# christoskokas/gtsam-vSLAM

Hardware: AMD Instinct MI355X
Metric: frames/sec (extract+match+localBA), 1500 feat stereo 752x480 (higher is better)
Workload: dtype u8/i32 (extract, match) + f64 (pose LM, local BA)

## Files before the change

### gtsam-vslam_amd/csrc/extract_kernels.hpp

```cpp
#pragma once
#include "common.hpp"

namespace vslam {

struct PyrDesc {
    int nLevels;
    int w[MAX_LEVELS], h[MAX_LEVELS], pitch[MAX_LEVELS];
    uint32_t off[MAX_LEVELS];
    uint32_t imgStride;
};

struct FastDesc {
    int minXY;
    int edge3;
    int nCols[MAX_LEVELS], nRows[MAX_LEVELS], gridW[MAX_LEVELS], gridH[MAX_LEVELS];
    int cellBase[MAX_LEVELS + 1];
    int cellCap;
    int tileRows, tilePitch;
};

struct BlurDesc {
    int tilesX[MAX_LEVELS];
    int tileBase[MAX_LEVELS + 1];
    int taps[7];
// ... 15 lines not shown
constexpr int FAST_TILE_MAX = 76;
constexpr int BLUR_RPT = 16;
constexpr int BLUR_TW = 256, BLUR_TH = 4 * BLUR_RPT;

void launch_load_images(hipStream_t s, const uint8_t* const* dSrc, int stride, uint8_t* pyr, const PyrDesc& P, int nimg);
void launch_load_images_color(hipStream_t s, const uint8_t* const* dSrc, int stride, int channels, uint8_t* pyr, const PyrDesc& P,
                              int nimg);
struct RectSrc {
    const uint8_t* src; const float* mapX; const float* mapY;
    int sw, sh, stride, pad;
};
void launch_load_images_rect(hipStream_t s, const RectSrc* dTab, int channels, uint8_t* pyr, const PyrDesc& P, int nimg);
void launch_resize(hipStream_t s, uint8_t* pyr, const PyrDesc& P, int level, const int2* xtab,
                   const int2* ytab, int nimg);
void launch_fast(hipStream_t s, const uint8_t* pyr, const PyrDesc& P, const FastDesc& F,
                 uint32_t* cellSlots, int* cellCount, int maxThr, int minThr, int nimg);
#ifdef VSLAM_FAST_CHECK
int fast_check_failures(hipStream_t s);
#endif
void launch_gather(hipStream_t s, const uint32_t* cellSlots, const int* cellCount, const FastDesc& F,
                   int nLevels, int* cellOff, uint32_t* cand, int candCap, int* levelCount, int nimg);
void launch_blur(hipStream_t s, const uint8_t* pyr, uint8_t* blur, const PyrDesc& P,
                 const BlurDesc& B, int nimg);
struct DiscRows { int umax[16]; };
void launch_orient_desc(hipStream_t s, const uint8_t* pyr, const uint8_t* blur, const PyrDesc& P,
                        const LevelTables& T, const uint32_t* kept, const int* keptOff, int keptCap,
                        const DiscRows& disc, vslam_keypoint* kps, uint8_t* desc, int outCap,
                        int maxKept, int nimg);
void upload_pattern();

constexpr int SSC_NMAX_LDS = 16384;
constexpr int SSC_NMAX = 65535;
constexpr int SSC_PICKW_G = 2048;
struct SscArgs {
    const uint32_t* cand; int candCap; const int* levelCount;
    int nLevels, nimg;
    int numRet[MAX_LEVELS], cols[MAX_LEVELS], rows[MAX_LEVELS], high[MAX_LEVELS], kmin[MAX_LEVELS], kmax[MAX_LEVELS];
    uint32_t* tmp;
    uint32_t* gridG;
    const size_t* gridOff;
    uint32_t* aG; uint32_t* sortedG; uint32_t* picksG;
    int forceGlobal;
    int* taskCount;
    int* flags;
};

void launch_ssc(hipStream_t s, const SscArgs& A, uint32_t* kept, int keptCap, int* keptOff, int* hostCounts);

}
```

### gtsam-vslam_amd/csrc/extractor.hip

```cpp
#include "extractor.hpp"
#include <atomic>
#include <algorithm>
#include <cmath>
#include <mutex>

namespace vslam {

static thread_local char g_err[512] = "";
void set_error(const char* fmt, ...) {
    va_list ap;
    va_start(ap, fmt);
    vsnprintf(g_err, sizeof(g_err), fmt, ap);
    va_end(ap);
}

}

using namespace vslam;

static void build_fe_tables(vslam_extractor& e) {
    const int nL = e.nLevels;
    const vslam_fe_params& p = e.prm;
    e.scalePyramid.assign(nL, 1.f);
    e.scaleInvPyramid.assign(nL, 1.f);
// ... 183 lines not shown
    VS_HIP(hipMalloc(&d_kept, (size_t)nimg * keptCap * sizeof(uint32_t)));
    VS_HIP(hipMalloc(&d_keptOff, (size_t)nimg * (MAX_LEVELS + 1) * sizeof(int)));
    VS_HIP(hipMalloc(&d_kps, (size_t)nimg * keptCap * sizeof(vslam_keypoint)));
    VS_HIP(hipMalloc(&d_desc, (size_t)nimg * keptCap * 32));

    for (int v = 0; v < 16; v++) discRows.umax[v] = umax[v];
    nKept.assign(nimg, 0);
    for (int l = 0; l < nLevels; l++) {
        const int numRet = featurePerLevel[l], cols = P.w[l], rows = P.h[l];
        const int e1 = rows + cols + 2 * numRet;
        const long long e2 = 4LL * cols + 4LL * numRet + 4LL * rows * numRet + (long long)rows * rows +
                             (long long)cols * cols - 2LL * rows * cols + 4LL * rows * cols * numRet;
        const double e3 = std::sqrt((double)e2), e4 = numRet - 1;
        const double s1 = -std::round((e1 + e3) / e4), s2 = -std::round((e1 - e3) / e4);
        sscHigh[l] = (int)(s1 > s2 ? s1 : s2);
        const unsigned K = (unsigned)numRet;
        sscKmin[l] = (int)(unsigned)std::round((float)K - ((float)K * 0.1f));
        sscKmax[l] = (int)(unsigned)std::round((float)K + ((float)K * 0.1f));
    }
    VS_HIP(hipMalloc(&d_sscTmp, (size_t)3 * nimg * candCap * sizeof(uint32_t)));
    VS_HIP(hipMalloc(&d_sscPicks, (size_t)nimg * nLevels * 8 * SSC_PICKW_G * sizeof(uint32_t)));
    {
        size_t words = 0;
        std::vector<size_t> off((size_t)nimg * nLevels, 0);
        for (int i = 0; i < nimg; i++)
            for (int l = 0; l < nLevels; l++) {
                off[(size_t)i * nLevels + l] = words;
                words += (size_t)(2 * P.h[l] + 2) * (size_t)((2 * P.w[l] + 2 + 31) / 32);
            }
        VS_HIP(hipMalloc(&d_sscGrid, words * sizeof(uint32_t)));
        VS_HIP(hipMalloc(&d_sscGridOff, off.size() * sizeof(size_t)));
        VS_HIP(hipMemcpy(d_sscGridOff, off.data(), off.size() * sizeof(size_t), hipMemcpyHostToDevice));
    }
    VS_HIP(hipMalloc(&d_taskCount, (size_t)nimg * MAX_LEVELS * sizeof(int) + (size_t)nimg * MAX_LEVELS * 8 * sizeof(long long)));
    VS_HIP(hipMalloc(&d_sscFlags, (size_t)nimg * 2 * sizeof(int)));
    VS_HIP(vslam::memset_sync(d_sscFlags, 0, (size_t)nimg * 2 * sizeof(int)));
    VS_HIP(hipHostMalloc(&h_counts, (size_t)nimg * 3 * sizeof(int), hipHostMallocMapped));
    VS_HIP(hipHostGetDevicePointer((void**)&d_counts, h_counts, 0));
    memset(h_counts, 0, (size_t)nimg * 3 * sizeof(int));
    if (const char* e = getenv("VSLAM_SSC_FORCE_GLOBAL")) sscForceGlobal = atoi(e) != 0;
    return VSLAM_OK;
}

void vslam_extractor::release() {
    if (stream) hipStreamSynchronize(stream);
    timer.destroy();
    hipFree(d_pyr); hipFree(d_blur); hipFree(d_xtab); hipFree(d_ytab);
    hipFree(d_cellSlots); hipFree(d_cellCount); hipFree(d_cellOff);
    hipFree(d_cand); hipFree(d_levelCount);
    if (doubleOut) { hipFree(d_kpsBuf[0]); hipFree(d_kpsBuf[1]); hipFree(d_descBuf[0]); hipFree(d_descBuf[1]); }
    else { hipFree(d_kps); hipFree(d_desc); }
    hipFree(d_kept); hipFree(d_keptOff);
    hipFree(d_sscTmp); hipFree(d_sscPicks); hipFree(d_taskCount); hipFree(d_sscFlags); hipFree(d_sscGrid); hipFree(d_sscGridOff);
    d_sscGrid = nullptr; d_sscGridOff = nullptr; d_sscPicks = nullptr;
    if (h_counts) hipHostFree(h_counts);
    if (h_imgPtrs) hipHostFree(h_imgPtrs);
    hipFree(d_imgPtrs); h_imgPtrs = nullptr; d_imgPtrs = nullptr;
    if (h_colPtrs) hipHostFree(h_colPtrs);
    hipFree(d_colPtrs); hipFree(d_colStage); h_colPtrs = nullptr; d_colPtrs = nullptr; d_colStage = nullptr; colStageBytes = 0;
    if (evColPtrs) hipEventDestroy(evColPtrs);
    evColPtrs = nullptr;
    if (h_rectTab) hipHostFree(h_rectTab);
    hipFree(d_rectTab); h_rectTab = nullptr; d_rectTab = nullptr;
    if (evRectTab) hipEventDestroy(evRectTab);
    evRectTab = nullptr;
    d_sscTmp = nullptr; d_taskCount = nullptr; d_sscFlags = nullptr; h_counts = nullptr;
    if (evGather) hipEventDestroy(evGather);
// ... 138 lines not shown
        hipFree(d_colStage); d_colStage = nullptr; colStageBytes = 0;
        VS_HIP(hipMalloc((void**)&d_colStage, need));
        colStageBytes = need;
    }
    size_t at = 0;
    for (int i = 0; i < nimg; i++) {
        RectSrc& t = h_rectTab[i];
        t = RectSrc{};
        if (!ptrs[i]) continue;
        const vslam_rectifier* r = rects[i];
        t.mapX = r->d_mapX; t.mapY = r->d_mapY; t.sw = r->sw; t.sh = r->sh;
        if (srcOnDevice) { t.src = ptrs[i]; t.stride = stride; continue; }
        const int pitch = align_up(r->sw * channels, 16);
        uint8_t* dst = d_colStage + at;
        at += (size_t)r->sh * pitch;
        VS_HIP(hipMemcpy2DAsync(dst, pitch, ptrs[i], stride, (size_t)r->sw * channels, r->sh, hipMemcpyHostToDevice, stream));
        t.src = dst; t.stride = pitch;
    }
    VS_HIP(hipMemcpyAsync(d_rectTab, h_rectTab, (size_t)nimg * sizeof(RectSrc), hipMemcpyHostToDevice, stream));
    VS_HIP(hipEventRecord(evRectTab, stream));
    launch_load_images_rect(stream, d_rectTab, channels, d_pyr, P, nimg);
    VS_HIP(hipGetLastError());
    if (sync && !srcOnDevice) VS_HIP(hipStreamSynchronize(stream));
    return VSLAM_OK;
}

vslam_status vslam_extractor::wait_counts() {
    if (!countsPending) return VSLAM_OK;
    VS_HIP(hipSetDevice(device));
    VS_HIP(hipEventSynchronize(evDone));
    countsPending = false;
#ifdef VSLAM_SSC_STAMPS
    {
        std::vector<long long> st((size_t)nimg * nLevels * 8);
        hipMemcpy(st.data(), d_taskCount + nimg * MAX_LEVELS, st.size() * sizeof(long long), hipMemcpyDeviceToHost);
        for (int i = 0; i < nimg; i++) for (int l = 0; l < nLevels; l++) { const long long* q = &st[(size_t)(i * nLevels + l) * 8]; fprintf(stderr, "ssc img %d lvl %d: n %lld partitions %lld countsort %lld search %lld (probes %lld final w %lld) emit %lld\n", i, l, q[4], q[0], q[1], q[2], q[5], q[6], q[3]); }
    }
#endif
    for (int i = 0; i < nimg; i++) {
        if (h_counts[nimg + 2 * i + 1]) { set_error("FAST candidate / kept-keypoint overflow"); return VSLAM_ERR_CAPACITY; }
        if (h_counts[nimg + 2 * i]) {
            set_error("SSC: image %d exceeds a kernel limit (mask %d: 1 = more than %d candidates in one level, 4 = segment list, "
                      "8 / 32 = width search, 16 = probe grid)", i, h_counts[nimg + 2 * i], SSC_NMAX);
            return VSLAM_ERR_CAPACITY;
        }
        nKept[i] = h_counts[i];
    }
    return VSLAM_OK;
}

vslam_status vslam_extractor::enqueue_ssc() {
    SscArgs S{};
    S.cand = d_cand; S.candCap = candCap; S.levelCount = d_levelCount; S.nLevels = nLevels; S.nimg = nimg;
    for (int l = 0; l < nLevels; l++) {
        S.numRet[l] = featurePerLevel[l]; S.cols[l] = P.w[l]; S.rows[l] = P.h[l];
        S.high[l] = sscHigh[l]; S.kmin[l] = sscKmin[l]; S.kmax[l] = sscKmax[l];
    }
    S.gridG = d_sscGrid; S.gridOff = d_sscGridOff;
    S.tmp = d_sscTmp; S.aG = d_sscTmp + (size_t)nimg * candCap; S.sortedG = d_sscTmp + (size_t)2 * nimg * candCap;
    S.picksG = d_sscPicks; S.forceGlobal = sscForceGlobal ? 1 : 0;
    S.taskCount = d_taskCount; S.flags = d_sscFlags;
    launch_ssc(stream, S, d_kept, keptCap, d_keptOff, d_counts);
    return VSLAM_OK;
}

#ifdef VSLAM_HOST_STAMPS
#include <chrono>
static double hs_now() { return std::chrono::duration<double, std::micro>(std::chrono::steady_clock::now().time_since_epoch()).count(); }
#define HS(k) hs[k] = hs_now()
// ... 296 lines not shown
```

### gtsam-vslam_amd/csrc/ssc.hip

```cpp
#include "extract_kernels.hpp"
#include <mutex>

namespace vslam {

constexpr int SSC_NT = 512, SSC_NW = SSC_NT / 64;
constexpr int SSC_NPROBE = 8;
constexpr int SSC_COOP_MIN = 2048;
constexpr int SSC_ARENA_WORDS = 20 * 1024;
constexpr int SSC_NMAX_SMALL = 6144;

template <int M> struct SscCfg;
template <> struct SscCfg<0> { static constexpr int NMAX = SSC_NMAX_LDS, SEGMAX = 1088, PICKW = SSC_NMAX_LDS / 32, ARENA = SSC_ARENA_WORDS; };
template <> struct SscCfg<1> { static constexpr int NMAX = SSC_NMAX, SEGMAX = 4096, PICKW = SSC_PICKW_G, ARENA = SSC_ARENA_WORDS; };
template <> struct SscCfg<2> { static constexpr int NMAX = SSC_NMAX_SMALL, SEGMAX = 1088, PICKW = SSC_NMAX_SMALL / 32, ARENA = 10 * 1024; };

template <bool G> __device__ __forceinline__ void ssc_fence() {
    if (G) asm volatile("s_waitcnt vmcnt(0) lgkmcnt(0)" ::: "memory");
    else asm volatile("s_waitcnt lgkmcnt(0)" ::: "memory");
}
__device__ __forceinline__ void ssc_lds_fence() { asm volatile("s_waitcnt lgkmcnt(0)" ::: "memory"); }

__device__ __forceinline__ int ssc_cell(int v, int width, float rcpw) {
    const int t = 2 * v;
    int q = (int)((float)t * rcpw);
    q -= (q * width > t);
    q += ((q + 1) * width <= t);
    return q;
}

template <bool G>
__device__ __forceinline__ int ssc_eval(const uint32_t* sc, int n, int width, int cols, int rows, uint32_t* grid, int gridWords,
                                        uint32_t* picks, bool& fits, int abortAbove) {
    const int lane = threadIdx.x & 63;
    const float rcpw = 1.0f / (float)width;
    const int gc = ssc_cell(cols, width, rcpw), gr = ssc_cell(rows, width, rcpw);
    const int span = 2;
    const int rowWords = (gc + 1 + 31) >> 5;
    const int words = (gr + 1) * rowWords;
    fits = words <= gridWords;
    if (!fits) return -1;
    for (int i = lane; i < words; i += 64) grid[i] = 0;
    ssc_lds_fence();
    asm volatile("s_waitcnt vmcnt(0)" ::: "memory");
    int count = 0;
    uint32_t pkNext = lane < n ? sc[lane] : 0u;
    for (int base = 0; base < n; base += 64) {
        const int i = base + lane;
        const bool valid = i < n;
        const uint32_t pk = pkNext;
        if (G) pkNext = (i + 64 < n) ? sc[i + 64] : 0u;
        const int row = ssc_cell(cand_y(pk), width, rcpw);
        const int col = ssc_cell(cand_x(pk), width, rcpw);
        bool covered = true;
        if (valid) covered = (grid[row * rowWords + (col >> 5)] >> (col & 31)) & 1u;
        unsigned long long pend = __ballot(!covered), picked = 0ull;
        while (pend) {
            const int l = __ffsll((long long)pend) - 1;
            picked |= 1ull << l;
            const int rl = __builtin_amdgcn_readlane(row, l), cl = __builtin_amdgcn_readlane(col, l);
            const bool conflict = abs(row - rl) <= span && abs(col - cl) <= span;
            pend &= ~__ballot(conflict);
        }
        if ((picked >> lane) & 1ull) {
            const int r0 = max(row - span, 0), r1 = min(row + span, gr);
            const int c0 = max(col - span, 0), c1 = min(col + span, gc);
            const int w0 = c0 >> 5, w1 = c1 >> 5;
            for (int rr = r0; rr <= r1; rr++) {
                if (w0 == w1) {
                    const uint32_t m = ((1u << (c1 - c0 + 1)) - 1u) << (c0 & 31);
                    atomicOr(&grid[rr * rowWords + w0], m);
                } else {
                    atomicOr(&grid[rr * rowWords + w0], 0xffffffffu << (c0 & 31));
                    atomicOr(&grid[rr * rowWords + w1], 0xffffffffu >> (31 - (c1 & 31)));
                }
            }
        }
        if (picks && lane < 2) picks[(base >> 5) + lane] = (uint32_t)(picked >> (32 * lane));
        count += __popcll(picked);
        if (!G) pkNext = (i + 64 < n) ? sc[i + 64] : 0u;
        ssc_lds_fence();
        asm volatile("s_waitcnt vmcnt(0)" ::: "memory");
        if (abortAbove >= 0 && count > abortAbove) break;
    }
    return count;
}

constexpr int SSC_LONGMAX = 64;
__device__ int g_sscCoopMin = SSC_COOP_MIN;
__device__ __forceinline__ void ssc_push(uint32_t* segN, int* cntN, int segMax, int f, int e, int depth, int* sFail) {
    if (e - f > g_sscCoopMin) {
        const int q = atomicAdd(cntN + 2, 1);
        if (q < SSC_LONGMAX) { segN[2 * q] = (uint32_t)f | ((uint32_t)e << 16); segN[2 * q + 1] = (uint32_t)depth; }
        else *sFail = 4;
        return;
    }
    const int q = atomicAdd(cntN, 1) + SSC_LONGMAX;
    if (q < segMax) { segN[2 * q] = (uint32_t)f | ((uint32_t)e << 16); segN[2 * q + 1] = (uint32_t)depth; }
    else *sFail = 4;
}

template <bool G>
__device__ void ssc_adjust_heap(uint32_t* first, int holeIndex, int len, uint32_t value) {
    const int topIndex = holeIndex;
    int secondChild = holeIndex;
    while (secondChild < (len - 1) / 2) {
        secondChild = 2 * (secondChild + 1);
        if ((first[secondChild] >> 16) < (first[secondChild - 1] >> 16)) secondChild--;
        first[holeIndex] = first[secondChild];
        ssc_fence<G>();
        holeIndex = secondChild;
    }
    if ((len & 1) == 0 && secondChild == (len - 2) / 2) {
        secondChild = 2 * (secondChild + 1);
        first[holeIndex] = first[secondChild - 1];
// ... 11 lines not shown
    ssc_fence<G>();
}
template <bool G>
__device__ void ssc_heapsort(uint32_t* first, int len) {
    if (len < 2) return;
    for (int parent = (len - 2) / 2;; parent--) {
        const uint32_t value = first[parent];
        ssc_adjust_heap<G>(first, parent, len, value);
        if (parent == 0) break;
    }
    for (int last = len; last > 1;) {
        --last;
        const uint32_t value = first[last];
        first[last] = first[0];
        ssc_fence<G>();
        ssc_adjust_heap<G>(first, 0, last, value);
    }
}

__device__ __forceinline__ int ssc_sel_lo(unsigned long long m, int k) {
    unsigned w = (unsigned)m;
    int pos = 0;
    const int cl = __popc(w);
    if (k >= cl) { k -= cl; w = (unsigned)(m >> 32); pos = 32; }
#pragma unroll
    for (int s = 16; s >= 1; s >>= 1) {
        const unsigned lowmask = (1u << s) - 1u;
        const int c = __popc(w & lowmask);
        if (k >= c) { k -= c; w >>= s; pos += s; } else w &= lowmask;
    }
    return pos;
}

template <bool G>
__device__ __forceinline__ void ssc_small_segment(uint32_t* a, int f, int e, int depth, uint16_t* Lp, uint16_t* Rp,
                                                  uint32_t* segN, int* cntN, int segMax, int* sFail) {
    const int lane = threadIdx.x & 63, m = e - f;
    uint32_t v = lane < m ? a[f + lane] : 0u;
    int lo = lane < m ? 0 : 64, hi = lane < m ? m : 64, d = depth;
    for (;;) {
        const bool act = (hi - lo) > 16;
        if (__ballot(act) == 0ull) break;
        if (__ballot(act && d == 0) != 0ull) {
            if (lane < m) a[f + lane] = v;
            if (act && lane == lo) ssc_push(segN, cntN, segMax, f + lo, f + hi, d, sFail);
            ssc_fence<G>();
            return;
        }
        const int ia = act ? lo + 1 : lane, ib = act ? lo + (hi - lo) / 2 : lane, ic = act ? hi - 1 : lane;
        const uint32_t va = __shfl(v, ia), vb = __shfl(v, ib), vc = __shfl(v, ic), vlo = __shfl(v, act ? lo : lane);
        const uint32_t ka = va >> 16, kb = vb >> 16, kc = vc >> 16;
        int mi;
        if (ka < kb) { if (kb < kc) mi = ib; else if (ka < kc) mi = ic; else mi = ia; }
        else if (ka < kc) mi = ia; else if (kb < kc) mi = ic; else mi = ib;
        const uint32_t vm = mi == ia ? va : (mi == ib ? vb : vc);
        if (act) { if (lane == lo) v = vm; else if (lane == mi) v = vlo; }
        const uint32_t pk = vm >> 16;
        const bool inR = act && lane > lo && lane < hi;
        const uint32_t kx = v >> 16;
        const bool isL = inR && kx >= pk, isR = inR && kx <= pk;
        const unsigned long long below = hi >= 64 ? ~0ull : ((1ull << hi) - 1ull);
        const unsigned long long segmask = act ? (below & ~((1ull << lo) - 1ull)) : 0ull;
        const unsigned long long mL = __ballot(isL) & segmask, mR = __ballot(isR) & segmask;
        const int nL = __popcll(mL), nR = __popcll(mR);
        const int kL = __popcll(mL & ((1ull << lane) - 1ull));
        const int kR = lane == 63 ? 0 : __popcll(mR >> (lane + 1));
        if (isL) Lp[f + lo + kL] = (uint16_t)lane;
        if (isR) Rp[f + lo + kR] = (uint16_t)lane;
        ssc_fence<G>();
        int src = lane;
        bool asL = false;
        if (isL && kL < nR) { const int p = Rp[f + lo + kL]; if (lane < p) { src = p; asL = true; } }
        if (!asL && isR && kR < nL) { const int p = Lp[f + lo + kR]; if (p < lane) src = p; }
        const int K = __popcll(__ballot(asL) & segmask);
        v = __shfl(v, src);
        if (act) {
            int cut = K >= 1 ? (int)Rp[f + lo + K - 1] : hi;
            if (K < nL) cut = min(cut, (int)Lp[f + lo + K]);
            d--;
            if (lane < cut) hi = cut; else lo = cut;
        }
        ssc_fence<G>();
    }
    if (lane < m) a[f + lane] = v;
    ssc_fence<G>();
}

__device__ __forceinline__ void ssc_median_to_first(uint32_t* a, int f, int e) {
    const int ia = f + 1, ib = f + (e - f) / 2, ic = e - 1;
    const uint32_t ka = a[ia] >> 16, kb = a[ib] >> 16, kc = a[ic] >> 16;
    int m;
    if (ka < kb) { if (kb < kc) m = ib; else if (ka < kc) m = ic; else m = ia; }
    else if (ka < kc) m = ia; else if (kb < kc) m = ic; else m = ib;
    const uint32_t t = a[f]; a[f] = a[m]; a[m] = t;
}

template <bool G>
__device__ __forceinline__ void ssc_partition_coop(uint32_t* a, uint16_t* Lp, uint16_t* Rp, int f, int e, int depth, int* sW,
                                                   uint32_t* segN, int* cntN, int segMax, int* sFail) {
    const int tid = threadIdx.x, lane = tid & 63, wave = tid >> 6;
    if (tid == 0) { ssc_median_to_first(a, f, e); ssc_fence<G>(); }
    __syncthreads();
    const uint32_t pk = a[f] >> 16;
    const int m = e - f - 1;
    const int per = ((m + SSC_NW - 1) / SSC_NW + 63) & ~63;
    const int c0 = min(e, f + 1 + wave * per), c1 = min(e, c0 + per);
    int nl = 0, nr = 0;
    for (int base = c0; base < c1; base += 64) {
        const int x = base + lane;
        const bool v = x < c1;
        const uint32_t kx = v ? (a[x] >> 16) : 0u;
        nl += __popcll(__ballot(v && kx >= pk)); nr += __popcll(__ballot(v && kx <= pk));
    }
    if (lane == 0) { sW[wave] = nl; sW[SSC_NW + wave] = nr; }
    __syncthreads();
    int offL = 0, offR = 0, nL = 0, nR = 0;
#pragma unroll
    for (int w = 0; w < SSC_NW; w++) {
        const int l = sW[w], r = sW[SSC_NW + w];
        if (w < wave) { offL += l; offR += r; }
        nL += l; nR += r;
    }
    const unsigned long long lt = (1ull << lane) - 1ull;
    for (int base = c0; base < c1; base += 64) {
        const int x = base + lane;
        const bool v = x < c1;
        const uint32_t kx = v ? (a[x] >> 16) : 0u;
// ... 23 lines not shown
    }
    ssc_fence<G>();
    __syncthreads();
}

template <int M>
__global__ __launch_bounds__(SSC_NT, 4) void k_ssc(SscArgs A) {
    using C = SscCfg<M>;
    constexpr bool G = M == 1;
    extern __shared__ uint32_t lds[];
    const int img = blockIdx.x % A.nimg, l = blockIdx.x / A.nimg;
    const int task = img * A.nLevels + l;
    const int* lc = A.levelCount + (size_t)img * (MAX_LEVELS + 1);
    int coff = 0;
    for (int q = 0; q < l; q++) coff += lc[q];
    const int n = lc[l];
    const int mode = (A.forceGlobal || n > SSC_NMAX_LDS) ? 1 : (n > SSC_NMAX_SMALL ? 0 : 2);
    if (mode != M) return;
    uint32_t* sortedU = G ? A.sortedG + (size_t)img * A.candCap + coff : lds;
    uint32_t* a = G ? A.aG + (size_t)img * A.candCap + coff : lds + C::NMAX;
    uint16_t* Lp = (uint16_t*)sortedU;
    uint16_t* Rp = Lp + (G ? n : C::NMAX);
    uint32_t* seg = G ? lds : lds + 2 * C::NMAX;
    uint32_t* arena = G ? lds + 4 * C::SEGMAX : lds + C::NMAX;
    int* h2 = G ? (int*)arena : (int*)seg;
    __shared__ int hist[256], sCnt[4], sFail, sW[2 * SSC_NW + 2];
    __shared__ int cacheW[64], cacheC[64], cacheSlot[64], nCache, sched[8], nSched, sFinal, sDone, sSolo;
    __shared__ int sLow, sHigh, sPrev, sLast;
    __shared__ int pre[C::PICKW];
    const int tid = threadIdx.x, lane = tid & 63;
    const int wave = __builtin_amdgcn_readfirstlane(tid >> 6);
#ifdef VSLAM_SSC_STAMPS
    long long st_t = clock64();
    long long* st = (long long*)(A.taskCount + A.nimg * MAX_LEVELS) + (size_t)task * 8;
#define SSC_STAMP(k) do { if (tid == 0) { const long long n_ = clock64(); st[k] = n_ - st_t; st_t = n_; } } while (0)
#else
#define SSC_STAMP(k) do {} while (0)
#endif
    const uint32_t* cand = A.cand + (size_t)img * A.candCap + coff;
    uint32_t* out = A.tmp + (size_t)img * A.candCap + coff;
    int* taskCount = A.taskCount + task;
    if (lc[MAX_LEVELS] > A.candCap) { if (tid == 0) { A.flags[2 * img + 1] = 1; *taskCount = 0; } return; }
    const int numRet = A.numRet[l];
    if (n <= numRet) {
        for (int i = tid; i < n; i += SSC_NT) out[i] = cand[i];
        if (tid == 0) *taskCount = n;
        return;
    }
    if (n > C::NMAX) { if (tid == 0) { atomicOr(&A.flags[2 * img], 1); *taskCount = 0; } return; }

    for (int i = tid; i < n; i += SSC_NT) a[i] = ((uint32_t)cand_s(cand[i]) << 16) | (uint32_t)i;
    if (tid < 256) hist[tid] = 0;
    if (tid == 0) {
        sFail = 0;
        int lg = 0;
        while ((1 << (lg + 1)) <= n) lg++;
        sCnt[0] = sCnt[1] = sCnt[2] = sCnt[3] = 0;
        if (n > 16) ssc_push(seg, &sCnt[0], C::SEGMAX, 0, n, 2 * lg, &sFail);
    }
    ssc_fence<G>();
    __syncthreads();
    int cur = 0;
    for (;;) {
        const int nseg = min(sCnt[cur], C::SEGMAX - SSC_LONGMAX), nlong = min(sCnt[2 + cur], SSC_LONGMAX);
        if (nseg == 0 && nlong == 0) break;
        const uint32_t* segL = seg + cur * C::SEGMAX * 2;
        const uint32_t* segC = segL + 2 * SSC_LONGMAX;
        uint32_t* segN = seg + (cur ^ 1) * C::SEGMAX * 2;
        int* cntN = &sCnt[cur ^ 1];
        for (int s = 0; s < nlong; s++) {
            const int f = (int)(segL[2 * s] & 0xffffu), e = (int)(segL[2 * s] >> 16), depth = (int)segL[2 * s + 1];
            if (depth == 0) { if (tid == 0) ssc_heapsort<G>(a + f, e - f); continue; }
            ssc_partition_coop<G>(a, Lp, Rp, f, e, depth, sW, segN, cntN, C::SEGMAX, &sFail);
        }
        for (int s = wave; s < nseg; s += SSC_NW) {
            const uint32_t sfe = (uint32_t)__builtin_amdgcn_readfirstlane((int)segC[2 * s]);
            const int f = (int)(sfe & 0xffffu), e = (int)(sfe >> 16), depth = __builtin_amdgcn_readfirstlane((int)segC[2 * s + 1]);
            if (depth == 0) { if (lane == 0) ssc_heapsort<G>(a + f, e - f); continue; }
            if (e - f <= 64) {
                ssc_small_segment<G>(a, f, e, depth, Lp, Rp, segN, cntN, C::SEGMAX, &sFail);
                continue;
            }
            if (lane == 0) ssc_median_to_first(a, f, e);
            ssc_fence<G>();
            const uint32_t pk = a[f] >> 16;
            int nL = 0, nR = 0;
            for (int base = f + 1; base < e; base += 64) {
                const int x = base + lane;
                const bool v = x < e;
                const uint32_t kx = v ? (a[x] >> 16) : 0u;
                const bool isL = v && kx >= pk, isR = v && kx <= pk;
                const unsigned long long bl = __ballot(isL), br = __ballot(isR);
                const unsigned long long lt = (1ull << lane) - 1ull;
                if (isL) Lp[f + 1 + nL + __popcll(bl & lt)] = (uint16_t)x;
                if (isR) Rp[f + 1 + nR + __popcll(br & lt)] = (uint16_t)x;
                nL += __popcll(bl); nR += __popcll(br);
            }
            ssc_fence<G>();
            const int nPair = min(nL, nR);
            int K = 0;
            for (int base = 0; base < nPair; base += 64) {
                const int k = base + lane;
                const bool ok = k < nPair && Lp[f + 1 + k] < Rp[f + 1 + nR - 1 - k];
                const unsigned long long bo = __ballot(ok);
                K += __popcll(bo);
                if (bo != ~0ull) break;
            }
            for (int k = lane; k < K; k += 64) {
                const int xl = Lp[f + 1 + k], xr = Rp[f + 1 + nR - 1 - k];
                const uint32_t t = a[xl]; a[xl] = a[xr]; a[xr] = t;
            }
            ssc_fence<G>();
            int cut = K >= 1 ? (int)Rp[f + 1 + nR - K] : e;
            if (K < nL) cut = min(cut, (int)Lp[f + 1 + K]);
            if (lane == 0) {
                if (e - cut > 16) ssc_push(segN, cntN, C::SEGMAX, cut, e, depth - 1, &sFail);
                if (cut - f > 16) ssc_push(segN, cntN, C::SEGMAX, f, cut, depth - 1, &sFail);
            }
        }
        ssc_fence<G>();
        __syncthreads();
        if (tid == 0) { sCnt[cur] = 0; sCnt[2 + cur] = 0; }
        cur ^= 1;
        __syncthreads();
    }
    SSC_STAMP(0);
    if (sFail) { if (tid == 0) { atomicOr(&A.flags[2 * img], sFail); *taskCount = 0; } return; }
    for (int i = tid; i < SSC_NW * 256; i += SSC_NT) h2[i] = 0;
    __syncthreads();
    const int per = ((n + SSC_NW - 1) / SSC_NW + 63) & ~63;
    const int s0 = min(n, wave * per), s1 = min(n, s0 + per);
    for (int i = s0 + lane; i < s1; i += 64) atomicAdd(&h2[wave * 256 + (int)(a[i] >> 16)], 1);
    __syncthreads();
    if (tid < 256) { int t = 0; for (int w = 0; w < SSC_NW; w++) t += h2[w * 256 + tid]; hist[tid] = t; }
    __syncthreads();
    if (wave == 0) {
        int run = 0;
        for (int base = 0; base < 256; base += 64) {
            const int v = hist[base + lane];
            int incl = v;
#pragma unroll
            for (int d = 1; d < 64; d <<= 1) { const int t = __shfl_up(incl, d); if (lane >= d) incl += t; }
            hist[base + lane] = run + incl - v;
            run += __shfl(incl, 63);
        }
    }
    __syncthreads();
    if (tid < 256) { int run = hist[tid]; for (int w = 0; w < SSC_NW; w++) { const int t = h2[w * 256 + tid]; h2[w * 256 + tid] = run; run += t; } }
    __syncthreads();
    {
        int* off = h2 + wave * 256;
        for (int base = s0; base < s1; base += 64) {
            const int i = base + lane;
            const bool v = i < s1;
// ... 5 lines not shown
                const unsigned long long bb = __ballot(v && ((key >> bit) & 1));
                same &= ((key >> bit) & 1) ? bb : ~bb;
            }
            same &= __ballot(v);
            if (v) {
                const int rank = __popcll(same & ((1ull << lane) - 1ull));
                sortedU[n - 1 - (off[key] + rank)] = cand[e & 0xffffu];
            }
            ssc_lds_fence();
            if (v && (same >> lane) == 1ull) off[key] += __popcll(same);
            ssc_lds_fence();
        }
    }
    ssc_fence<G>();
    __syncthreads();
    SSC_STAMP(1);
    const uint32_t* sc = sortedU;

    if (tid == 0) {
        sLow = max(1, (int)floor(sqrt((double)n / numRet)));
        sHigh = A.high[l]; sPrev = -1; sLast = -1; nCache = 0; sDone = 0; sFinal = -1; sSolo = 0;
    }
    __syncthreads();
    const int kmin = A.kmin[l], kmax = A.kmax[l];
    const int cols = A.cols[l], rows = A.rows[l];
    uint32_t* gridG = A.gridG + A.gridOff[task];
    constexpr int SLICE = C::ARENA / SSC_NPROBE;
    uint32_t* picksG = G ? A.picksG + (size_t)task * SSC_NPROBE * SSC_PICKW_G : nullptr;
    constexpr int PICKW_L = G ? 0 : C::PICKW;
    auto picks_of = [&](int slot) -> uint32_t* {
        if (G) return picksG + (size_t)(slot < 0 ? SSC_NPROBE - 1 : slot) * SSC_PICKW_G;
        return slot < 0 ? arena + C::ARENA - PICKW_L : arena + slot * SLICE + SLICE - PICKW_L;
    };
    for (int round = 0; round < 64; round++) {
        if (tid == 0) {
            nSched = 0;
            for (;;) {
                const int width = sLow + (sHigh - sLow) / 2;
                if (width == sPrev || sLow > sHigh) { sFinal = sLast; sDone = 1; break; }
                int cnt = -1;
                for (int q = 0; q < nCache; q++) if (cacheW[q] == width) cnt = cacheC[q];
                if (cnt < 0) break;
                sLast = width;
                if (cnt >= kmin && cnt <= kmax) { sFinal = width; sDone = 1; break; }
                if (cnt < kmin) sHigh = width - 1; else sLow = width + 1;
                sPrev = width;
            }
            if (!sDone) {
                int qlow[8], qhigh[8], qprev[8];
                qlow[1] = sLow; qhigh[1] = sHigh; qprev[1] = sPrev;
                for (int node = 1; node < 8; node++) {
                    const int lo = qlow[node], hi = qhigh[node], pv = qprev[node];
                    const int width = lo + (hi - lo) / 2;
                    const bool term = lo > hi || width == pv;
                    if (!term) {
                        bool dup = false;
                        for (int q = 0; q < nSched; q++) dup |= sched[q] == width;
                        for (int q = 0; q < nCache; q++) dup |= cacheW[q] == width;
                        if (!dup && nSched < SSC_NPROBE - 1) sched[nSched++] = width;
                    }
                    if (2 * node + 1 < 8) {
                        qlow[2 * node] = term ? 1 : lo; qhigh[2 * node] = term ? 0 : width - 1; qprev[2 * node] = width;
                        qlow[2 * node + 1] = term ? 1 : width + 1; qhigh[2 * node + 1] = term ? 0 : hi; qprev[2 * node + 1] = width;
                    }
                }
                if (sSolo) nSched = 1;
            }
// ... 123 lines not shown
```

Measured before the change: 28930.

## Restructure SSC quicksort partitioning into multi-wave subtrees and batch grid probes

Replaces the single-wave small-segment sort with a templated subtree sorter that handles segments of up to 128 or 256 elements across several register slots, doing the partition steps in LDS or global memory. Larger segments now go through a rewritten one-wave partition that fuses the swap pass with the pair search and pushes both children with one atomic. The SSC probe loop also checks grid coverage four chunks at a time while nothing is picked, and only fences after a chunk that picked something. This cuts per-level synchronisation and serial lane-0 work, at the cost of more complex index bookkeeping, higher register pressure, and new timing stamps that are compiled only under a debug flag.

```diff
diff --git a/gtsam-vslam_amd/csrc/extract_kernels.hpp b/gtsam-vslam_amd/csrc/extract_kernels.hpp
--- a/gtsam-vslam_amd/csrc/extract_kernels.hpp
+++ b/gtsam-vslam_amd/csrc/extract_kernels.hpp
@@ -71,6 +71,12 @@
 constexpr int SSC_NMAX_LDS = 16384;
 constexpr int SSC_NMAX = 65535;
 constexpr int SSC_PICKW_G = 2048;
+#ifdef VSLAM_SSC_STAMPS
+constexpr int SSC_STAMP_LEVELS = 24, SSC_STAMP_ROUNDS = 24;
+constexpr int SSC_STAMP_SLOTS = 8 + 4 * SSC_STAMP_LEVELS + SSC_STAMP_ROUNDS;
+#else
+constexpr int SSC_STAMP_SLOTS = 8;
+#endif
 struct SscArgs {
     const uint32_t* cand; int candCap; const int* levelCount;
     int nLevels, nimg;
diff --git a/gtsam-vslam_amd/csrc/extractor.hip b/gtsam-vslam_amd/csrc/extractor.hip
--- a/gtsam-vslam_amd/csrc/extractor.hip
+++ b/gtsam-vslam_amd/csrc/extractor.hip
@@ -239,7 +239,7 @@
         VS_HIP(hipMalloc(&d_sscGridOff, off.size() * sizeof(size_t)));
         VS_HIP(hipMemcpy(d_sscGridOff, off.data(), off.size() * sizeof(size_t), hipMemcpyHostToDevice));
     }
-    VS_HIP(hipMalloc(&d_taskCount, (size_t)nimg * MAX_LEVELS * sizeof(int) + (size_t)nimg * MAX_LEVELS * 8 * sizeof(long long)));
+    VS_HIP(hipMalloc(&d_taskCount, (size_t)nimg * MAX_LEVELS * sizeof(int) + (size_t)nimg * MAX_LEVELS * SSC_STAMP_SLOTS * sizeof(long long)));
     VS_HIP(hipMalloc(&d_sscFlags, (size_t)nimg * 2 * sizeof(int)));
     VS_HIP(vslam::memset_sync(d_sscFlags, 0, (size_t)nimg * 2 * sizeof(int)));
     VS_HIP(hipHostMalloc(&h_counts, (size_t)nimg * 3 * sizeof(int), hipHostMallocMapped));
@@ -444,9 +444,18 @@
     countsPending = false;
 #ifdef VSLAM_SSC_STAMPS
     {
-        std::vector<long long> st((size_t)nimg * nLevels * 8);
+        std::vector<long long> st((size_t)nimg * nLevels * SSC_STAMP_SLOTS);
         hipMemcpy(st.data(), d_taskCount + nimg * MAX_LEVELS, st.size() * sizeof(long long), hipMemcpyDeviceToHost);
-        for (int i = 0; i < nimg; i++) for (int l = 0; l < nLevels; l++) { const long long* q = &st[(size_t)(i * nLevels + l) * 8]; fprintf(stderr, "ssc img %d lvl %d: n %lld partitions %lld countsort %lld search %lld (probes %lld final w %lld) emit %lld\n", i, l, q[4], q[0], q[1], q[2], q[5], q[6], q[3]); }
+        for (int i = 0; i < nimg; i++) for (int l = 0; l < nLevels; l++) {
+            const long long* q = &st[(size_t)(i * nLevels + l) * SSC_STAMP_SLOTS];
+            fprintf(stderr, "ssc img %d lvl %d: n %lld partitions %lld countsort %lld search %lld (probes %lld final w %lld) emit %lld\n", i, l, q[4], q[0], q[1], q[2], q[5], q[6], q[3]);
+            if (i == 0 && l == 0) {
+                for (int t = 0; t < SSC_STAMP_LEVELS && (q[8 + 4 * t] || q[9 + 4 * t]); t++)
+                    fprintf(stderr, "  tree level %2d: coop %6lld  short %6lld  (one-wave max %6lld, sub-tree max %6lld)\n", t, q[8 + 4 * t], q[9 + 4 * t], q[10 + 4 * t], q[11 + 4 * t]);
+                for (int r = 0; r < SSC_STAMP_ROUNDS && q[8 + 4 * SSC_STAMP_LEVELS + r]; r++)
+                    fprintf(stderr, "  search round %2d: %6lld\n", r, q[8 + 4 * SSC_STAMP_LEVELS + r]);
+            }
+        }
     }
 #endif
     for (int i = 0; i < nimg; i++) {
diff --git a/gtsam-vslam_amd/csrc/ssc.hip b/gtsam-vslam_amd/csrc/ssc.hip
--- a/gtsam-vslam_amd/csrc/ssc.hip
+++ b/gtsam-vslam_amd/csrc/ssc.hip
@@ -10,9 +10,15 @@
 constexpr int SSC_NMAX_SMALL = 6144;
 
 template <int M> struct SscCfg;
-template <> struct SscCfg<0> { static constexpr int NMAX = SSC_NMAX_LDS, SEGMAX = 1088, PICKW = SSC_NMAX_LDS / 32, ARENA = SSC_ARENA_WORDS; };
-template <> struct SscCfg<1> { static constexpr int NMAX = SSC_NMAX, SEGMAX = 4096, PICKW = SSC_PICKW_G, ARENA = SSC_ARENA_WORDS; };
-template <> struct SscCfg<2> { static constexpr int NMAX = SSC_NMAX_SMALL, SEGMAX = 1088, PICKW = SSC_NMAX_SMALL / 32, ARENA = 10 * 1024; };
+#ifndef VSLAM_SSC_TREE_MAX
+#define VSLAM_SSC_TREE_MAX 256
+#endif
+#ifndef VSLAM_SSC_TREE_MAX_SMALL
+#define VSLAM_SSC_TREE_MAX_SMALL 128
+#endif
+template <> struct SscCfg<0> { static constexpr int NMAX = SSC_NMAX_LDS, SEGMAX = 1088, PICKW = SSC_NMAX_LDS / 32, ARENA = SSC_ARENA_WORDS, TREE = VSLAM_SSC_TREE_MAX; };
+template <> struct SscCfg<1> { static constexpr int NMAX = SSC_NMAX, SEGMAX = 4096, PICKW = SSC_PICKW_G, ARENA = SSC_ARENA_WORDS, TREE = VSLAM_SSC_TREE_MAX; };
+template <> struct SscCfg<2> { static constexpr int NMAX = SSC_NMAX_SMALL, SEGMAX = 1088, PICKW = SSC_NMAX_SMALL / 32, ARENA = 10 * 1024, TREE = VSLAM_SSC_TREE_MAX_SMALL; };
 
 template <bool G> __device__ __forceinline__ void ssc_fence() {
     if (G) asm volatile("s_waitcnt vmcnt(0) lgkmcnt(0)" ::: "memory");
@@ -43,17 +49,8 @@
     ssc_lds_fence();
     asm volatile("s_waitcnt vmcnt(0)" ::: "memory");
     int count = 0;
-    uint32_t pkNext = lane < n ? sc[lane] : 0u;
-    for (int base = 0; base < n; base += 64) {
-        const int i = base + lane;
-        const bool valid = i < n;
-        const uint32_t pk = pkNext;
-        if (G) pkNext = (i + 64 < n) ? sc[i + 64] : 0u;
-        const int row = ssc_cell(cand_y(pk), width, rcpw);
-        const int col = ssc_cell(cand_x(pk), width, rcpw);
-        bool covered = true;
-        if (valid) covered = (grid[row * rowWords + (col >> 5)] >> (col & 31)) & 1u;
-        unsigned long long pend = __ballot(!covered), picked = 0ull;
+    auto resolve = [&](int base, int row, int col, unsigned long long pend) {
+        unsigned long long picked = 0ull;
         while (pend) {
             const int l = __ffsll((long long)pend) - 1;
             picked |= 1ull << l;
@@ -77,9 +74,55 @@
         }
         if (picks && lane < 2) picks[(base >> 5) + lane] = (uint32_t)(picked >> (32 * lane));
         count += __popcll(picked);
-        if (!G) pkNext = (i + 64 < n) ? sc[i + 64] : 0u;
-        ssc_lds_fence();
-        asm volatile("s_waitcnt vmcnt(0)" ::: "memory");
+        if (picked) {
+            ssc_lds_fence();
+            asm volatile("s_waitcnt vmcnt(0)" ::: "memory");
+        }
+    };
+    constexpr int SSC_BATCH = 4;
+    bool batch = false;
+    uint32_t pkNext = lane < n ? sc[lane] : 0u;
+    for (int base = 0; base < n;) {
+        if (!batch) {
+            const int i = base + lane;
+            const uint32_t pk = pkNext;
+            const int row = ssc_cell(cand_y(pk), width, rcpw);
+            const int col = ssc_cell(cand_x(pk), width, rcpw);
+            bool covered = true;
+            if (i < n) covered = (grid[row * rowWords + (col >> 5)] >> (col & 31)) & 1u;
+            pkNext = (i + 64 < n) ? sc[i + 64] : 0u;
+            const unsigned long long pend = __ballot(!covered);
+            resolve(base, row, col, pend);
+            batch = pend == 0ull;
+            base += 64;
+        } else {
+            int row[SSC_BATCH], col[SSC_BATCH];
+            bool covered[SSC_BATCH];
+#pragma unroll
+            for (int q = 0; q < SSC_BATCH; q++) {
+                const int i = base + 64 * q + lane;
+                const uint32_t pk = q == 0 ? pkNext : (i < n ? sc[i] : 0u);
+                row[q] = ssc_cell(cand_y(pk), width, rcpw);
+                col[q] = ssc_cell(cand_x(pk), width, rcpw);
+            }
+#pragma unroll
+            for (int q = 0; q < SSC_BATCH; q++) {
+                covered[q] = true;
+                if (base + 64 * q + lane < n) covered[q] = (grid[row[q] * rowWords + (col[q] >> 5)] >> (col[q] & 31)) & 1u;
+            }
+            int qf = min(SSC_BATCH, (n - base + 63) >> 6), rowf = 0, colf = 0;
+            unsigned long long pend = 0ull;
+#pragma unroll
+            for (int q = SSC_BATCH - 1; q >= 0; q--) {
+                const unsigned long long u = __ballot(!covered[q]);
+                if (u) { qf = q; pend = u; rowf = row[q]; colf = col[q]; }
+            }
+            const int next = base + 64 * (qf + (pend ? 1 : 0));
+            pkNext = next + lane < n ? sc[next + lane] : 0u;
+            if (picks && lane < 2 * qf) picks[(base >> 5) + lane] = 0u;
+            if (pend) { resolve(base + 64 * qf, rowf, colf, pend); batch = false; }
+            base = next;
+        }
         if (abortAbove >= 0 && count > abortAbove) break;
     }
     return count;
@@ -157,57 +200,116 @@
     return pos;
 }
 
-template <bool G>
-__device__ __forceinline__ void ssc_small_segment(uint32_t* a, int f, int e, int depth, uint16_t* Lp, uint16_t* Rp,
-                                                  uint32_t* segN, int* cntN, int segMax, int* sFail) {
+template <bool G, int E>
+__device__ __forceinline__ void ssc_subtree(uint32_t* a, int f, int e, int depth, uint16_t* Lp, uint16_t* Rp,
+                                            uint32_t* segN, int* cntN, int segMax, int* sFail) {
+    static_assert(E <= 4, "the end counts of a sub-segment are kept in 8 bits");
     const int lane = threadIdx.x & 63, m = e - f;
-    uint32_t v = lane < m ? a[f + lane] : 0u;
-    int lo = lane < m ? 0 : 64, hi = lane < m ? m : 64, d = depth;
-    for (;;) {
-        const bool act = (hi - lo) > 16;
-        if (__ballot(act) == 0ull) break;
-        if (__ballot(act && d == 0) != 0ull) {
-            if (lane < m) a[f + lane] = v;
-            if (act && lane == lo) ssc_push(segN, cntN, segMax, f + lo, f + hi, d, sFail);
-            ssc_fence<G>();
-            return;
-        }
-        const int ia = act ? lo + 1 : lane, ib = act ? lo + (hi - lo) / 2 : lane, ic = act ? hi - 1 : lane;
-        const uint32_t va = __shfl(v, ia), vb = __shfl(v, ib), vc = __shfl(v, ic), vlo = __shfl(v, act ? lo : lane);
-        const uint32_t ka = va >> 16, kb = vb >> 16, kc = vc >> 16;
-        int mi;
-        if (ka < kb) { if (kb < kc) mi = ib; else if (ka < kc) mi = ic; else mi = ia; }
-        else if (ka < kc) mi = ia; else if (kb < kc) mi = ic; else mi = ib;
-        const uint32_t vm = mi == ia ? va : (mi == ib ? vb : vc);
-        if (act) { if (lane == lo) v = vm; else if (lane == mi) v = vlo; }
-        const uint32_t pk = vm >> 16;
-        const bool inR = act && lane > lo && lane < hi;
-        const uint32_t kx = v >> 16;
-        const bool isL = inR && kx >= pk, isR = inR && kx <= pk;
-        const unsigned long long below = hi >= 64 ? ~0ull : ((1ull << hi) - 1ull);
-        const unsigned long long segmask = act ? (below & ~((1ull << lo) - 1ull)) : 0ull;
-        const unsigned long long mL = __ballot(isL) & segmask, mR = __ballot(isR) & segmask;
-        const int nL = __popcll(mL), nR = __popcll(mR);
-        const int kL = __popcll(mL & ((1ull << lane) - 1ull));
-        const int kR = lane == 63 ? 0 : __popcll(mR >> (lane + 1));
-        if (isL) Lp[f + lo + kL] = (uint16_t)lane;
-        if (isR) Rp[f + lo + kR] = (uint16_t)lane;
-        ssc_fence<G>();
-        int src = lane;
-        bool asL = false;
-        if (isL && kL < nR) { const int p = Rp[f + lo + kL]; if (lane < p) { src = p; asL = true; } }
-        if (!asL && isR && kR < nL) { const int p = Lp[f + lo + kR]; if (p < lane) src = p; }
-        const int K = __popcll(__ballot(asL) & segmask);
-        v = __shfl(v, src);
-        if (act) {
-            int cut = K >= 1 ? (int)Rp[f + lo + K - 1] : hi;
-            if (K < nL) cut = min(cut, (int)Lp[f + lo + K]);
-            d--;
-            if (lane < cut) hi = cut; else lo = cut;
-        }
-        ssc_fence<G>();
-    }
-    if (lane < m) a[f + lane] = v;
+    uint32_t* as = a + f;
+    uint16_t* L = Lp + f;
+    uint16_t* R = Rp + f;
+    uint32_t v[E];
+    int lo[E], hi[E];
+#pragma unroll
+    for (int c = 0; c < E; c++) {
+        const int j = 64 * c + lane;
+        v[c] = j < m ? as[j] : 0u;
+        lo[c] = j < m ? 0 : j; hi[c] = j < m ? m : j;
+    }
+    for (int d = depth;; d--) {
+        bool act[E], any = false;
+#pragma unroll
+        for (int c = 0; c < E; c++) { act[c] = hi[c] - lo[c] > 16; any |= act[c]; }
+        if (__ballot(any) == 0ull) break;
+        if (d == 0) {
+#pragma unroll
+            for (int c = 0; c < E; c++) if (act[c] && 64 * c + lane == lo[c]) ssc_push(segN, cntN, segMax, f + lo[c], f + hi[c], 0, sFail);
+            break;
+        }
+        uint32_t va[E], vb[E], vc[E], vl[E];
+#pragma unroll
+        for (int c = 0; c < E; c++) {
+            const int l0 = act[c] ? lo[c] : 0, h0 = act[c] ? hi[c] : 2;
+            va[c] = as[l0 + 1]; vb[c] = as[l0 + (h0 - l0) / 2]; vc[c] = as[h0 - 1]; vl[c] = as[l0];
+        }
+        ssc_fence<G>();
+        bool isL[E], isR[E];
+        int PL[E], PR[E];
+        int baseL = 0, baseR = 0;
+#pragma unroll
+        for (int c = 0; c < E; c++) {
+            const int j = 64 * c + lane, ia = lo[c] + 1, ib = lo[c] + (hi[c] - lo[c]) / 2, ic = hi[c] - 1;
+            const uint32_t ka = va[c] >> 16, kb = vb[c] >> 16, kc = vc[c] >> 16;
+            int mi;
+            if (ka < kb) { if (kb < kc) mi = ib; else if (ka < kc) mi = ic; else mi = ia; }
+            else if (ka < kc) mi = ia; else if (kb < kc) mi = ic; else mi = ib;
+            const uint32_t vm = mi == ia ? va[c] : (mi == ib ? vb[c] : vc[c]);
+            if (act[c]) {
+                if (j == lo[c]) { as[lo[c]] = vm; as[mi] = vl[c]; v[c] = vm; }
+                else if (j == mi) v[c] = vl[c];
+            }
+            const uint32_t pk = vm >> 16, kx = v[c] >> 16;
+            const bool inR = act[c] && j > lo[c] && j < hi[c];
+            isL[c] = inR && kx >= pk; isR[c] = inR && kx <= pk;
+            const unsigned long long bl = __ballot(isL[c]), br = __ballot(isR[c]);
+            PL[c] = baseL + (int)__builtin_amdgcn_mbcnt_hi((uint32_t)(bl >> 32), __builtin_amdgcn_mbcnt_lo((uint32_t)bl, 0u));
+            PR[c] = baseR + (int)__builtin_amdgcn_mbcnt_hi((uint32_t)(br >> 32), __builtin_amdgcn_mbcnt_lo((uint32_t)br, 0u));
+            baseL += __popcll(bl); baseR += __popcll(br);
+            if (act[c] && j == lo[c]) L[hi[c] - 1] = (uint16_t)(PL[c] | (PR[c] << 8));
+            if (act[c] && j == hi[c] - 1) R[hi[c] - 1] = (uint16_t)((PL[c] + (int)isL[c]) | ((PR[c] + (int)isR[c]) << 8));
+        }
+        ssc_fence<G>();
+        int endL[E], endR[E];
+#pragma unroll
+        for (int c = 0; c < E; c++) { endL[c] = act[c] ? (int)L[hi[c] - 1] : 0; endR[c] = act[c] ? (int)R[hi[c] - 1] : 0; }
+        ssc_fence<G>();
+        int kL[E], kR[E], nL[E], nR[E];
+#pragma unroll
+        for (int c = 0; c < E; c++) {
+            nL[c] = (endR[c] & 255) - (endL[c] & 255); nR[c] = (endR[c] >> 8) - (endL[c] >> 8);
+            kL[c] = PL[c] - (endL[c] & 255);
+            kR[c] = (endR[c] >> 8) - PR[c] - 1;
+            if (isL[c]) L[lo[c] + kL[c]] = (uint16_t)(64 * c + lane);
+            if (isR[c]) R[lo[c] + kR[c]] = (uint16_t)(64 * c + lane);
+        }
+        ssc_fence<G>();
+        int pR[E], pL[E], qL[E], qR[E];
+#pragma unroll
+        for (int c = 0; c < E; c++) {
+            pR[c] = (isL[c] && kL[c] < nR[c]) ? (int)R[lo[c] + kL[c]] : -1;
+            pL[c] = (isR[c] && kR[c] < nL[c]) ? (int)L[lo[c] + kR[c]] : 64 * E;
+            qL[c] = (isL[c] && kL[c] >= 1) ? (int)L[lo[c] + kL[c] - 1] : 0;
+            qR[c] = (isL[c] && kL[c] >= 1 && kL[c] - 1 < nR[c]) ? (int)R[lo[c] + kL[c] - 1] : -1;
+        }
+        ssc_fence<G>();
+        int src[E];
+#pragma unroll
+        for (int c = 0; c < E; c++) {
+            const int j = 64 * c + lane;
+            const bool asL = j < pR[c];
+            src[c] = asL ? pR[c] : (pL[c] < j ? pL[c] : j);
+            const bool prevPass = kL[c] >= 1 ? qL[c] < qR[c] : true;
+            if (isL[c] && !asL && prevPass) L[hi[c] - 1] = (uint16_t)min(kL[c] >= 1 ? qR[c] : hi[c], j);
+            else if (isL[c] && asL && kL[c] == nL[c] - 1) L[hi[c] - 1] = (uint16_t)pR[c];
+        }
+        ssc_fence<G>();
+        uint32_t nv[E];
+        int cut[E];
+#pragma unroll
+        for (int c = 0; c < E; c++) {
+            nv[c] = src[c] != 64 * c + lane ? as[src[c]] : v[c];
+            cut[c] = act[c] ? (int)L[hi[c] - 1] : 0;
+        }
+        ssc_fence<G>();
+#pragma unroll
+        for (int c = 0; c < E; c++) {
+            const int j = 64 * c + lane;
+            if (src[c] != j) as[j] = nv[c];
+            v[c] = nv[c];
+            if (act[c]) { if (j < cut[c]) hi[c] = cut[c]; else lo[c] = cut[c]; }
+        }
+        ssc_fence<G>();
+    }
     ssc_fence<G>();
 }
 
@@ -218,6 +320,67 @@
     if (ka < kb) { if (kb < kc) m = ib; else if (ka < kc) m = ic; else m = ia; }
     else if (ka < kc) m = ia; else if (kb < kc) m = ic; else m = ib;
     const uint32_t t = a[f]; a[f] = a[m]; a[m] = t;
+}
+
+__device__ __forceinline__ void ssc_push_children(uint32_t* segN, int* cntN, int segMax, int f, int cut, int e, int depth, int* sFail) {
+    const bool r = e - cut > 16, l = cut - f > 16;
+    if (!r && !l) return;
+    int q = atomicAdd(cntN, (int)r + (int)l) + SSC_LONGMAX;
+    if (q + (int)r + (int)l > segMax) { *sFail = 4; return; }
+    if (r) { segN[2 * q] = (uint32_t)cut | ((uint32_t)e << 16); segN[2 * q + 1] = (uint32_t)depth; q++; }
+    if (l) { segN[2 * q] = (uint32_t)f | ((uint32_t)cut << 16); segN[2 * q + 1] = (uint32_t)depth; }
+}
+
+template <bool G>
+__device__ __forceinline__ void ssc_partition_wave(uint32_t* a, uint16_t* Lp, uint16_t* Rp, int f, int e, int depth,
+                                                   uint32_t* segN, int* cntN, int segMax, int* sFail) {
+    const int lane = threadIdx.x & 63;
+    const int i4 = lane == 0 ? f + 1 : (lane == 1 ? f + (e - f) / 2 : (lane == 2 ? e - 1 : f));
+    const uint32_t v4 = a[i4];
+    const uint32_t va = (uint32_t)__builtin_amdgcn_readlane((int)v4, 0), vb = (uint32_t)__builtin_amdgcn_readlane((int)v4, 1);
+    const uint32_t vc = (uint32_t)__builtin_amdgcn_readlane((int)v4, 2), vf = (uint32_t)__builtin_amdgcn_readlane((int)v4, 3);
+    const uint32_t ka = va >> 16, kb = vb >> 16, kc = vc >> 16;
+    int ms;
+    if (ka < kb) { if (kb < kc) ms = 1; else if (ka < kc) ms = 2; else ms = 0; }
+    else if (ka < kc) ms = 0; else if (kb < kc) ms = 2; else ms = 1;
+    const uint32_t vm = ms == 0 ? va : (ms == 1 ? vb : vc);
+    if (lane == ms) a[i4] = vf;
+    if (lane == 3) a[f] = vm;
+    ssc_fence<G>();
+    const uint32_t pk = vm >> 16;
+    int nL = 0, nR = 0;
+    const unsigned long long lt = (1ull << lane) - 1ull;
+    for (int base = f + 1; base < e; base += 64) {
+        const int x = base + lane;
+        const bool v = x < e;
+        const uint32_t kx = v ? (a[x] >> 16) : 0u;
+        const bool isL = v && kx >= pk, isR = v && kx <= pk;
+        const unsigned long long bl = __ballot(isL), br = __ballot(isR);
+        if (isL) Lp[f + 1 + nL + __popcll(bl & lt)] = (uint16_t)x;
+        if (isR) Rp[f + 1 + nR + __popcll(br & lt)] = (uint16_t)x;
+        nL += __popcll(bl); nR += __popcll(br);
+    }
+    ssc_fence<G>();
+    const int nPair = min(nL, nR);
+    int K = 0, cut = e, xrPrev = e;
+    for (int base = 0;; base += 64) {
+        const int k = base + lane;
+        const int xl = k < nL ? (int)Lp[f + 1 + k] : e, xr = k < nR ? (int)Rp[f + 1 + nR - 1 - k] : f;
+        const bool ok = k < nPair && xl < xr;
+        const unsigned long long bo = __ballot(ok);
+        if (ok) { const uint32_t tl = a[xl], tr = a[xr]; a[xl] = tr; a[xr] = tl; }
+        if (bo != ~0ull) {
+            const int kk = __popcll(bo);
+            K += kk;
+            if (K >= 1) cut = kk >= 1 ? __builtin_amdgcn_readlane(xr, kk - 1) : xrPrev;
+            if (K < nL) cut = min(cut, __builtin_amdgcn_readlane(xl, kk));
+            break;
+        }
+        K += 64;
+        xrPrev = __builtin_amdgcn_readlane(xr, 63);
+    }
+    if (lane == 0) ssc_push_children(segN, cntN, segMax, f, cut, e, depth - 1, sFail);
+    ssc_fence<G>();
 }
 
 template <bool G>
@@ -307,10 +470,17 @@
     const int wave = __builtin_amdgcn_readfirstlane(tid >> 6);
 #ifdef VSLAM_SSC_STAMPS
     long long st_t = clock64();
-    long long* st = (long long*)(A.taskCount + A.nimg * MAX_LEVELS) + (size_t)task * 8;
+    long long* st = (long long*)(A.taskCount + A.nimg * MAX_LEVELS) + (size_t)task * SSC_STAMP_SLOTS;
+    for (int i = 8 + tid; i < SSC_STAMP_SLOTS; i += SSC_NT) st[i] = 0;
+    long long st_u = st_t;
+    int st_lev = 0;
 #define SSC_STAMP(k) do { if (tid == 0) { const long long n_ = clock64(); st[k] = n_ - st_t; st_t = n_; } } while (0)
+#define SSC_STAMP_D(k) do { if (tid == 0 && (k) < SSC_STAMP_SLOTS) { const long long n_ = clock64(); st[k] = n_ - st_u; st_u = n_; } } while (0)
+#define SSC_STAMP_W(k, c) do { if (lane == 0 && (k) < SSC_STAMP_SLOTS) atomicMax((unsigned long long*)&st[k], (unsigned long long)(c)); } while (0)
 #else
 #define SSC_STAMP(k) do {} while (0)
+#define SSC_STAMP_D(k) do {} while (0)
+#define SSC_STAMP_W(k, c) do {} while (0)
 #endif
     const uint32_t* cand = A.cand + (size_t)img * A.candCap + coff;
     uint32_t* out = A.tmp + (size_t)img * A.candCap + coff;
@@ -336,6 +506,9 @@
     ssc_fence<G>();
     __syncthreads();
     int cur = 0;
+#ifdef VSLAM_SSC_STAMPS
+    st_u = clock64();
+#endif
     for (;;) {
         const int nseg = min(sCnt[cur], C::SEGMAX - SSC_LONGMAX), nlong = min(sCnt[2 + cur], SSC_LONGMAX);
         if (nseg == 0 && nlong == 0) break;
@@ -348,53 +521,31 @@
             if (depth == 0) { if (tid == 0) ssc_heapsort<G>(a + f, e - f); continue; }
             ssc_partition_coop<G>(a, Lp, Rp, f, e, depth, sW, segN, cntN, C::SEGMAX, &sFail);
         }
+#ifdef VSLAM_SSC_STAMPS
+        if (st_lev < SSC_STAMP_LEVELS) SSC_STAMP_D(8 + 4 * st_lev);
+        long long st_one = 0, st_tree = 0;
+#endif
         for (int s = wave; s < nseg; s += SSC_NW) {
             const uint32_t sfe = (uint32_t)__builtin_amdgcn_readfirstlane((int)segC[2 * s]);
             const int f = (int)(sfe & 0xffffu), e = (int)(sfe >> 16), depth = __builtin_amdgcn_readfirstlane((int)segC[2 * s + 1]);
             if (depth == 0) { if (lane == 0) ssc_heapsort<G>(a + f, e - f); continue; }
-            if (e - f <= 64) {
-                ssc_small_segment<G>(a, f, e, depth, Lp, Rp, segN, cntN, C::SEGMAX, &sFail);
-                continue;
-            }
-            if (lane == 0) ssc_median_to_first(a, f, e);
-            ssc_fence<G>();
-            const uint32_t pk = a[f] >> 16;
-            int nL = 0, nR = 0;
-            for (int base = f + 1; base < e; base += 64) {
-                const int x = base + lane;
-                const bool v = x < e;
-                const uint32_t kx = v ? (a[x] >> 16) : 0u;
-                const bool isL = v && kx >= pk, isR = v && kx <= pk;
-                const unsigned long long bl = __ballot(isL), br = __ballot(isR);
-                const unsigned long long lt = (1ull << lane) - 1ull;
-                if (isL) Lp[f + 1 + nL + __popcll(bl & lt)] = (uint16_t)x;
-                if (isR) Rp[f + 1 + nR + __popcll(br & lt)] = (uint16_t)x;
-                nL += __popcll(bl); nR += __popcll(br);
-            }
-            ssc_fence<G>();
-            const int nPair = min(nL, nR);
-            int K = 0;
-            for (int base = 0; base < nPair; base += 64) {
-                const int k = base + lane;
-                const bool ok = k < nPair && Lp[f + 1 + k] < Rp[f + 1 + nR - 1 - k];
-                const unsigned long long bo = __ballot(ok);
-                K += __popcll(bo);
-                if (bo != ~0ull) break;
-            }
-            for (int k = lane; k < K; k += 64) {
-                const int xl = Lp[f + 1 + k], xr = Rp[f + 1 + nR - 1 - k];
-                const uint32_t t = a[xl]; a[xl] = a[xr]; a[xr] = t;
-            }
-            ssc_fence<G>();
-            int cut = K >= 1 ? (int)Rp[f + 1 + nR - K] : e;
-            if (K < nL) cut = min(cut, (int)Lp[f + 1 + K]);
-            if (lane == 0) {
-                if (e - cut > 16) ssc_push(segN, cntN, C::SEGMAX, cut, e, depth - 1, &sFail);
-                if (cut - f > 16) ssc_push(segN, cntN, C::SEGMAX, f, cut, depth - 1, &sFail);
-            }
+#ifdef VSLAM_SSC_STAMPS
+            const long long st_s = clock64();
+#endif
+            if (e - f <= 64) ssc_subtree<G, 1>(a, f, e, depth, Lp, Rp, segN, cntN, C::SEGMAX, &sFail);
+            else if (C::TREE >= 128 && e - f <= 128) ssc_subtree<G, 2>(a, f, e, depth, Lp, Rp, segN, cntN, C::SEGMAX, &sFail);
+            else if (C::TREE >= 256 && e - f <= 256) ssc_subtree<G, 4>(a, f, e, depth, Lp, Rp, segN, cntN, C::SEGMAX, &sFail);
+            else ssc_partition_wave<G>(a, Lp, Rp, f, e, depth, segN, cntN, C::SEGMAX, &sFail);
+#ifdef VSLAM_SSC_STAMPS
+            if (e - f <= C::TREE) st_tree += clock64() - st_s; else st_one += clock64() - st_s;
+#endif
         }
         ssc_fence<G>();
         __syncthreads();
+#ifdef VSLAM_SSC_STAMPS
+        if (st_lev < SSC_STAMP_LEVELS) { SSC_STAMP_D(9 + 4 * st_lev); SSC_STAMP_W(10 + 4 * st_lev, st_one); SSC_STAMP_W(11 + 4 * st_lev, st_tree); }
+        st_lev++;
+#endif
         if (tid == 0) { sCnt[cur] = 0; sCnt[2 + cur] = 0; }
         cur ^= 1;
         __syncthreads();
@@ -466,7 +617,13 @@
         if (G) return picksG + (size_t)(slot < 0 ? SSC_NPROBE - 1 : slot) * SSC_PICKW_G;
         return slot < 0 ? arena + C::ARENA - PICKW_L : arena + slot * SLICE + SLICE - PICKW_L;
     };
+#ifdef VSLAM_SSC_STAMPS
+    st_u = clock64();
+#endif
     for (int round = 0; round < 64; round++) {
+#ifdef VSLAM_SSC_STAMPS
+        if (round > 0 && round <= SSC_STAMP_ROUNDS) SSC_STAMP_D(8 + 4 * SSC_STAMP_LEVELS + round - 1);
+#endif
         if (tid == 0) {
             nSched = 0;
             for (;;) {
```

After: 27860. 3.7% lower.
